# YannDubs/disentangling-vae

Measured on AMD Instinct MI355X. Metric: images/sec (whole node) at 64x64x3, btcvae loss, higher is better.
Workload: dtype f32; 1 GPU; btcvae_celeba (BASELINE.json configs[3]): Burgess VAE 64x64x3, btcvae loss, z=10, tensor handed to _train_iteration B=1024 global (1024 per GPU), Adam lr 0.0005, n_data=202599, fwd+loss+bwd+Adam; batch_per_gpu=1024, global_batch=1024, parallelism=dp1

## Files before the change

disentangling-vae_amd/csrc/conv_up_thin_mm.hip:

```cpp
#include "recon_epilogue.h"

namespace dvae {

#define UTM_ROWS 12
#define UTM_COLS 34
#define UTM_TILE (UTM_ROWS * UTM_COLS * 32)
#define UTM_BR 11
#define UTM_NPOS (UTM_BR * 33)
#define UTM_OR 22
#define UTM_STAGE (3 * UTM_OR * 64)

__device__ __forceinline__ float sigmoid_hw_mm(float v) { return sigmoid_aten(v); }

#ifndef UTM_VARIANT
#define UTM_VARIANT 13
#endif
#ifndef UTM_ABL
#define UTM_ABL 0
#endif
__device__ __forceinline__ void utm_barrier() {
  if (UTM_VARIANT & 4) { wait_lgkmcnt0(); barrier_nofence(); }
  else __syncthreads();
}

template <bool FUSE, int DIST, typename TT>
__global__ __launch_bounds__(512, 4) void k_up_thin_mm(const float* __restrict__ small, const float* __restrict__ wimg,
                                                       const float* __restrict__ bias, float* __restrict__ out, int N,
                                                       int n_units, const TT* __restrict__ target, float* __restrict__ g,
                                                       const float* __restrict__ coef, float* __restrict__ partials) {
  extern __shared__ __attribute__((aligned(16))) float smem[];
  float* tin = smem;
  float* stage = smem + UTM_TILE;
  float* redl = stage + UTM_STAGE;
  float* wl = redl + 8;
  const int tid = threadIdx.x, lane = tid & 63;
  const int wv = __builtin_amdgcn_readfirstlane(tid >> 6);
  const int j = lane & 15, kg = lane >> 4;
  const float gs = FUSE ? coef[DVAE_C_INV_B] : 0.f;
  float lsum = 0.f;

  for (int e = tid; e < UTM_TILE / 4; e += 512) reinterpret_cast<f32x4*>(tin)[e] = f32x4{0.f, 0.f, 0.f, 0.f};

  for (int e = tid; e < 32 * 64 / 4; e += 512) reinterpret_cast<f32x4*>(wl)[e] = reinterpret_cast<const f32x4*>(wimg)[e];
  const float bv = (kg < 3 && bias) ? bias[kg] : 0.f;

  int xb[3], soff[3];
  int key0[3];
  bool x0ok[3], x1ok[3];
#pragma unroll
  for (int s = 0; s < 3; ++s) {
    const int pos0 = 16 * (3 * wv + s) + j;
    const bool pvalid = pos0 < UTM_NPOS;
    const int pos = pvalid ? pos0 : UTM_NPOS - 1;
    const int rq = pos / 33, cq = pos - 33 * rq;
    xb[s] = (rq * UTM_COLS + cq) * 32;
    key0[s] = cq & 7;
    soff[s] = (kg * UTM_OR + 2 * rq) * 64 + 2 * cq - 1;
    x0ok[s] = pvalid && kg < 3 && cq > 0;
    x1ok[s] = pvalid && kg < 3 && cq < 32;
  }
  const bool tile3 = 16 * (3 * wv + 2) < UTM_NPOS;
  const int within = tid & 255, rhalf = tid >> 8;
  const int pgo = rhalf * 1024 + within * 4;
  const int ci_ld = (within >> 3) + 1;
  const int plo = (rhalf * UTM_COLS + ci_ld) * 32 + (((within & 7) ^ (ci_ld & 7)) << 2);
  int bso[3], bgo[3], brow[3];
#pragma unroll
  for (int k = 0; k < 3; ++k) {
    const int e = tid + 512 * k;
    const int c = e / (UTM_OR * 16), rem = e - c * (UTM_OR * 16), r = rem >> 4, x4 = rem & 15;
    brow[k] = e < 3 * UTM_OR * 16 ? r : -1000;
    bso[k] = (c * UTM_OR + r) * 64 + 4 * x4;
    bgo[k] = (c * 64 + r) * 64 + 4 * x4;
  }
  __syncthreads();

  f32x4 pf[6];
  auto load_tile = [&](int unit) {
    const int n = unit / 3, u3 = unit - 3 * n;
    const int sy0 = UTM_BR * u3 - 1;
    const float* base = small + ((long)n * 32 + sy0) * 1024 + pgo;
#pragma unroll
    for (int k = 0; k < 6; ++k) {
      const int sy = sy0 + 2 * k + rhalf;
      pf[k] = f32x4{0.f, 0.f, 0.f, 0.f};
      if (sy >= 0 && sy < 32 && !((UTM_ABL & 16) && N > 0)) pf[k] = *reinterpret_cast<const f32x4*>(base + 2048 * k);
    }
  };
  if ((int)blockIdx.x < n_units) load_tile(blockIdx.x);
  for (int unit = blockIdx.x; unit < n_units; unit += gridDim.x) {
    const int n = unit / 3, u3 = unit - 3 * n;
    const int Y0 = UTM_OR * u3 - 1;
    const long img0 = ((long)n * 3 * 64 + Y0) * 64;
    f32x4 tg[3];
    uchar4 tg8[3];
    auto load_targets_k = [&](int k) {
      const int Y = Y0 + brow[k];
      tg[k] = f32x4{0.f, 0.f, 0.f, 0.f};
      tg8[k] = make_uchar4(0, 0, 0, 0);
      if (Y >= 0 && Y < 64) {
        if constexpr (sizeof(TT) == 4) tg[k] = *reinterpret_cast<const f32x4*>(target + img0 + bgo[k]);
        else tg8[k] = *reinterpret_cast<const uchar4*>(target + img0 + bgo[k]);
      }
    };
    auto load_targets = [&]() {
#pragma unroll
      for (int k = 0; k < 3; ++k) {
        const int Y = Y0 + brow[k];
        tg[k] = f32x4{0.f, 0.f, 0.f, 0.f};
        tg8[k] = make_uchar4(0, 0, 0, 0);
        if (Y >= 0 && Y < 64 && !((UTM_ABL & 4) && N > 0)) {
          if constexpr (sizeof(TT) == 4) tg[k] = *reinterpret_cast<const f32x4*>(target + img0 + bgo[k]);
          else tg8[k] = *reinterpret_cast<const uchar4*>(target + img0 + bgo[k]);
        }
      }
    };
#pragma unroll
    for (int k = 0; k < 6; ++k) *reinterpret_cast<f32x4*>(tin + plo + 2 * UTM_COLS * 32 * k) = pf[k];
    if ((UTM_VARIANT & 1) && unit + (int)gridDim.x < n_units) load_tile(unit + gridDim.x);
    if (FUSE && (UTM_VARIANT & 2)) load_targets();
    if (FUSE && (UTM_VARIANT & 16)) load_targets_k(0);
    utm_barrier();
    f32x4 acc[3];
#pragma unroll
    for (int s = 0; s < 3; ++s) acc[s] = f32x4{0.f, 0.f, 0.f, 0.f};
#pragma unroll
    for (int tap = 0; tap < 4; ++tap) {
      const int a = tap >> 1, b = tap & 1;
      f32x4 x[3][2];
      float wr[8];
#pragma unroll
      for (int i = 0; i < 8; ++i) wr[i] = wl[(tap * 8 + i) * 64 + lane];
#pragma unroll
      for (int s = 0; s < 3; ++s) {
        if (s == 2 && !tile3) continue;
        const int key = (key0[s] + b) & 7;
        const float* px = tin + xb[s] + (a * UTM_COLS + b) * 32;
        x[s][0] = *reinterpret_cast<const f32x4*>(px + (((2 * kg) ^ key) << 2));
        x[s][1] = *reinterpret_cast<const f32x4*>(px + (((2 * kg + 1) ^ key) << 2));
      }
#pragma unroll
      for (int i = 0; i < 8; ++i) {
#pragma unroll
        for (int s = 0; s < 3; ++s) {
          if (s == 2 && !tile3) continue;
          if (!((UTM_ABL & 1) && N > 0)) acc[s] = __builtin_amdgcn_mfma_f32_16x16x4f32(wr[i], x[s][i >> 2][i & 3], acc[s], 0, 0, 0);
        }
      }
    }
    if (FUSE && (UTM_VARIANT & 8)) load_targets();
    if (FUSE && (UTM_VARIANT & 16)) { load_targets_k(1); load_targets_k(2); }
#pragma unroll
    for (int s = 0; s < 3; ++s) {
      if (s == 2 && !tile3) continue;
      float* sp = stage + soff[s];
      if (x0ok[s]) { sp[0] = acc[s][0] + bv; sp[64] = acc[s][2] + bv; }
      if (x1ok[s]) { sp[1] = acc[s][1] + bv; sp[65] = acc[s][3] + bv; }
    }
    utm_barrier();
    if (!(UTM_VARIANT & 1) && unit + (int)gridDim.x < n_units) load_tile(unit + gridDim.x);
    if (FUSE && !(UTM_VARIANT & (2 | 8 | 16))) load_targets();
    if (FUSE && sizeof(TT) != 4) {
#pragma unroll
      for (int k = 0; k < 3; ++k) tg[k] = f32x4{to_unit(tg8[k].x), to_unit(tg8[k].y), to_unit(tg8[k].z), to_unit(tg8[k].w)};
    }
#pragma unroll
    for (int k = 0; k < 3; ++k) {
      const int Y = Y0 + brow[k];
      if (Y < 0 || Y >= 64) continue;
      f32x4 v = *reinterpret_cast<const f32x4*>(stage + bso[k]);
      f32x4 gl = {0.f, 0.f, 0.f, 0.f};
#pragma unroll
      for (int q = 0; q < 4; ++q) {
        if ((UTM_ABL & 2) && N > 0) {
          gl[q] = v[q] + tg[k][q];
        } else if (FUSE && DIST == DVAE_REC_BERNOULLI) {
          float y, glq;
          lsum += sigmoid_bce_logit(v[q], tg[k][q], &y, &glq);
          v[q] = y;
          gl[q] = gs * glq;
        } else {
          const float y = sigmoid_hw_mm(v[q]);
          v[q] = y;
          if (FUSE) {
            float glq, gr;
            lsum += recon_elem(y, tg[k][q], DIST, &glq, &gr);
            gl[q] = gs * glq;
          }
        }
      }
      if ((UTM_ABL & 8) && N > 0) { lsum += v[0] + v[1] + v[2] + v[3] + gl[0] + gl[1] + gl[2] + gl[3]; continue; }
      *reinterpret_cast<f32x4*>(out + img0 + bgo[k]) = v;
      if (FUSE) *reinterpret_cast<f32x4*>(g + img0 + bgo[k]) = gl;
    }
  }
  if (FUSE) {
    const float v = wave_sum(lsum);
    __syncthreads();
    if (lane == 0) redl[wv] = v;
    __syncthreads();
    if (tid == 0) {
      float s = 0.f;
#pragma unroll
      for (int w = 0; w < 8; ++w) s += redl[w];
      partials[blockIdx.x] = s;
    }
    for (int k = gridDim.x + blockIdx.x * 512 + tid; k < DVAE_REC_NPART; k += gridDim.x * 512) partials[k] = 0.f;
  }
}

int launch_up_thin_mm(const float* small, const float* wimg, const float* bias, const void* target, int target_u8, float* out,
                      float* g, int dist, const float* coef, float* partials, int N, int act, hipStream_t s) {
  static const bool off = env_off("DVAE_UP_THIN_MM");
  static const int min_n = env_int("DVAE_UP_THIN_MM_MIN_N", 1);
  if (off || N < min_n || act != DVAE_ACT_SIGMOID) return 1;
  if ((((uintptr_t)small | (uintptr_t)out | (uintptr_t)g) & 15) != 0 || ((uintptr_t)target & (target_u8 ? 3 : 15)) != 0) return 1;
  const int n_units = 3 * N;
  static const int cap = env_int("DVAE_UP_THIN_MM_GRID", 512);
  const int grid = n_units < cap ? n_units : cap;
  constexpr size_t lds = (size_t)(UTM_TILE + UTM_STAGE + 8 + 32 * 64) * sizeof(float);
#define UTM_GO(FUSE_, DIST_, TT_)                                                                                         \
  do {                                                                                                                    \
    static DeviceOnce attr;                                                                                               \
    if (attr.first())                                                                                                     \
      (void)hipFuncSetAttribute((const void*)k_up_thin_mm<FUSE_, DIST_, TT_>, hipFuncAttributeMaxDynamicSharedMemorySize, (int)lds); \
    hipLaunchKernelGGL((k_up_thin_mm<FUSE_, DIST_, TT_>), dim3(grid), dim3(512), lds, s, small, wimg, bias, out, N, n_units,      \
                       (const TT_*)target, g, coef, partials);                                                           \
  } while (0)
  if (!target) UTM_GO(false, 0, float);
  else if (target_u8) {
    if (dist == DVAE_REC_BERNOULLI) UTM_GO(true, DVAE_REC_BERNOULLI, uint8_t);
    else if (dist == DVAE_REC_GAUSSIAN) UTM_GO(true, DVAE_REC_GAUSSIAN, uint8_t);
    else UTM_GO(true, DVAE_REC_LAPLACE, uint8_t);
  } else {
    if (dist == DVAE_REC_BERNOULLI) UTM_GO(true, DVAE_REC_BERNOULLI, float);
    else if (dist == DVAE_REC_GAUSSIAN) UTM_GO(true, DVAE_REC_GAUSSIAN, float);
    else UTM_GO(true, DVAE_REC_LAPLACE, float);
  }
#undef UTM_GO
  DVAE_CHECK_LAUNCH();
  return 0;
}

}
```

Before: 989,600 images/s.

## Stream input tiles into LDS via async DMA and hoist target loads

```diff
diff --git a/disentangling-vae_amd/csrc/conv_up_thin_mm.hip b/disentangling-vae_amd/csrc/conv_up_thin_mm.hip
--- a/disentangling-vae_amd/csrc/conv_up_thin_mm.hip
+++ b/disentangling-vae_amd/csrc/conv_up_thin_mm.hip
@@ -12,16 +12,13 @@
 
 __device__ __forceinline__ float sigmoid_hw_mm(float v) { return sigmoid_aten(v); }
 
-#ifndef UTM_VARIANT
-#define UTM_VARIANT 13
-#endif
+__device__ __attribute__((aligned(16))) float k_utm_zero16[4] = {0.f, 0.f, 0.f, 0.f};
 #ifndef UTM_ABL
 #define UTM_ABL 0
 #endif
-__device__ __forceinline__ void utm_barrier() {
-  if (UTM_VARIANT & 4) { wait_lgkmcnt0(); barrier_nofence(); }
-  else __syncthreads();
-}
+__device__ __forceinline__ void utm_barrier() { wait_lgkmcnt0(); barrier_nofence(); }
+__device__ __forceinline__ void utm_need(f32x4& v) { asm volatile("" : "+v"(v)); }
+__device__ __forceinline__ void utm_need(unsigned& v) { asm volatile("" : "+v"(v)); }
 
 template <bool FUSE, int DIST, typename TT>
 __global__ __launch_bounds__(512, 4) void k_up_thin_mm(const float* __restrict__ small, const float* __restrict__ wimg,
@@ -38,14 +35,11 @@
   const int j = lane & 15, kg = lane >> 4;
   const float gs = FUSE ? coef[DVAE_C_INV_B] : 0.f;
   float lsum = 0.f;
-
   for (int e = tid; e < UTM_TILE / 4; e += 512) reinterpret_cast<f32x4*>(tin)[e] = f32x4{0.f, 0.f, 0.f, 0.f};
-
   for (int e = tid; e < 32 * 64 / 4; e += 512) reinterpret_cast<f32x4*>(wl)[e] = reinterpret_cast<const f32x4*>(wimg)[e];
   const float bv = (kg < 3 && bias) ? bias[kg] : 0.f;
 
-  int xb[3], soff[3];
-  int key0[3];
+  int xb[3], soff[3], key0[3];
   bool x0ok[3], x1ok[3];
 #pragma unroll
   for (int s = 0; s < 3; ++s) {
@@ -60,10 +54,23 @@
     x1ok[s] = pvalid && kg < 3 && cq < 32;
   }
   const bool tile3 = 16 * (3 * wv + 2) < UTM_NPOS;
-  const int within = tid & 255, rhalf = tid >> 8;
-  const int pgo = rhalf * 1024 + within * 4;
-  const int ci_ld = (within >> 3) + 1;
-  const int plo = (rhalf * UTM_COLS + ci_ld) * 32 + (((within & 7) ^ (ci_ld & 7)) << 2);
+  const int dpx = lane >> 3;
+  const int dlo = dpx * 32 + (((lane & 7) ^ ((dpx + 1) & 7)) << 2);
+  const unsigned lds0 = (unsigned)(unsigned long long)(__attribute__((address_space(3))) void*)smem;
+  auto issue_tile = [&](int unit) {
+    if ((UTM_ABL & 16) && N > 0) return;
+    const int n = unit / 3, u3 = unit - 3 * n;
+    const int sy0 = UTM_BR * u3 - 1;
+    const float* base = small + ((long)n * 32 + sy0) * 1024 + dlo;
+#pragma unroll
+    for (int k = 0; k < 6; ++k) {
+      const int d = wv + 8 * k;
+      const int r = d >> 2, c8 = d & 3;
+      const int sy = sy0 + r;
+      const float* src = (sy >= 0 && sy < 32) ? base + r * 1024 + c8 * 256 : k_utm_zero16;
+      lds_dma16(src, __builtin_amdgcn_readfirstlane(lds0 + (unsigned)((r * UTM_COLS + 1 + 8 * c8) * 32) * 4u));
+    }
+  };
   int bso[3], bgo[3], brow[3];
 #pragma unroll
   for (int k = 0; k < 3; ++k) {
@@ -75,52 +82,25 @@
   }
   __syncthreads();
 
-  f32x4 pf[6];
-  auto load_tile = [&](int unit) {
-    const int n = unit / 3, u3 = unit - 3 * n;
-    const int sy0 = UTM_BR * u3 - 1;
-    const float* base = small + ((long)n * 32 + sy0) * 1024 + pgo;
-#pragma unroll
-    for (int k = 0; k < 6; ++k) {
-      const int sy = sy0 + 2 * k + rhalf;
-      pf[k] = f32x4{0.f, 0.f, 0.f, 0.f};
-      if (sy >= 0 && sy < 32 && !((UTM_ABL & 16) && N > 0)) pf[k] = *reinterpret_cast<const f32x4*>(base + 2048 * k);
-    }
-  };
-  if ((int)blockIdx.x < n_units) load_tile(blockIdx.x);
+  if ((int)blockIdx.x < n_units) issue_tile(blockIdx.x);
+  wait_vmcnt<0>();
+  utm_barrier();
   for (int unit = blockIdx.x; unit < n_units; unit += gridDim.x) {
     const int n = unit / 3, u3 = unit - 3 * n;
     const int Y0 = UTM_OR * u3 - 1;
     const long img0 = ((long)n * 3 * 64 + Y0) * 64;
     f32x4 tg[3];
-    uchar4 tg8[3];
-    auto load_targets_k = [&](int k) {
+    unsigned tg8[3];
+#pragma unroll
+    for (int k = 0; k < 3; ++k) {
       const int Y = Y0 + brow[k];
       tg[k] = f32x4{0.f, 0.f, 0.f, 0.f};
-      tg8[k] = make_uchar4(0, 0, 0, 0);
-      if (Y >= 0 && Y < 64) {
+      tg8[k] = 0u;
+      if (FUSE && Y >= 0 && Y < 64 && !((UTM_ABL & 4) && N > 0)) {
         if constexpr (sizeof(TT) == 4) tg[k] = *reinterpret_cast<const f32x4*>(target + img0 + bgo[k]);
-        else tg8[k] = *reinterpret_cast<const uchar4*>(target + img0 + bgo[k]);
-      }
-    };
-    auto load_targets = [&]() {
-#pragma unroll
-      for (int k = 0; k < 3; ++k) {
-        const int Y = Y0 + brow[k];
-        tg[k] = f32x4{0.f, 0.f, 0.f, 0.f};
-        tg8[k] = make_uchar4(0, 0, 0, 0);
-        if (Y >= 0 && Y < 64 && !((UTM_ABL & 4) && N > 0)) {
-          if constexpr (sizeof(TT) == 4) tg[k] = *reinterpret_cast<const f32x4*>(target + img0 + bgo[k]);
-          else tg8[k] = *reinterpret_cast<const uchar4*>(target + img0 + bgo[k]);
-        }
-      }
-    };
-#pragma unroll
-    for (int k = 0; k < 6; ++k) *reinterpret_cast<f32x4*>(tin + plo + 2 * UTM_COLS * 32 * k) = pf[k];
-    if ((UTM_VARIANT & 1) && unit + (int)gridDim.x < n_units) load_tile(unit + gridDim.x);
-    if (FUSE && (UTM_VARIANT & 2)) load_targets();
-    if (FUSE && (UTM_VARIANT & 16)) load_targets_k(0);
-    utm_barrier();
+        else tg8[k] = *reinterpret_cast<const unsigned*>(target + img0 + bgo[k]);
+      }
+    }
     f32x4 acc[3];
 #pragma unroll
     for (int s = 0; s < 3; ++s) acc[s] = f32x4{0.f, 0.f, 0.f, 0.f};
@@ -148,8 +128,6 @@
         }
       }
     }
-    if (FUSE && (UTM_VARIANT & 8)) load_targets();
-    if (FUSE && (UTM_VARIANT & 16)) { load_targets_k(1); load_targets_k(2); }
 #pragma unroll
     for (int s = 0; s < 3; ++s) {
       if (s == 2 && !tile3) continue;
@@ -157,42 +135,59 @@
       if (x0ok[s]) { sp[0] = acc[s][0] + bv; sp[64] = acc[s][2] + bv; }
       if (x1ok[s]) { sp[1] = acc[s][1] + bv; sp[65] = acc[s][3] + bv; }
     }
+    if (FUSE) {
+#pragma unroll
+      for (int k = 0; k < 3; ++k) {
+        if constexpr (sizeof(TT) == 4) utm_need(tg[k]);
+        else utm_need(tg8[k]);
+      }
+    }
     utm_barrier();
-    if (!(UTM_VARIANT & 1) && unit + (int)gridDim.x < n_units) load_tile(unit + gridDim.x);
-    if (FUSE && !(UTM_VARIANT & (2 | 8 | 16))) load_targets();
+    if (unit + (int)gridDim.x < n_units) issue_tile(unit + gridDim.x);
     if (FUSE && sizeof(TT) != 4) {
 #pragma unroll
-      for (int k = 0; k < 3; ++k) tg[k] = f32x4{to_unit(tg8[k].x), to_unit(tg8[k].y), to_unit(tg8[k].z), to_unit(tg8[k].w)};
-    }
+      for (int k = 0; k < 3; ++k)
+        tg[k] = f32x4{to_unit((uint8_t)(tg8[k] & 0xff)), to_unit((uint8_t)((tg8[k] >> 8) & 0xff)), to_unit((uint8_t)((tg8[k] >> 16) & 0xff)),
+                      to_unit((uint8_t)(tg8[k] >> 24))};
+    }
+    f32x4 v[3], gl[3];
+    bool on[3];
 #pragma unroll
     for (int k = 0; k < 3; ++k) {
       const int Y = Y0 + brow[k];
-      if (Y < 0 || Y >= 64) continue;
-      f32x4 v = *reinterpret_cast<const f32x4*>(stage + bso[k]);
-      f32x4 gl = {0.f, 0.f, 0.f, 0.f};
+      on[k] = Y >= 0 && Y < 64;
+      v[k] = gl[k] = f32x4{0.f, 0.f, 0.f, 0.f};
+      if (!on[k]) continue;
+      v[k] = *reinterpret_cast<const f32x4*>(stage + bso[k]);
 #pragma unroll
       for (int q = 0; q < 4; ++q) {
         if ((UTM_ABL & 2) && N > 0) {
-          gl[q] = v[q] + tg[k][q];
+          gl[k][q] = v[k][q] + tg[k][q];
         } else if (FUSE && DIST == DVAE_REC_BERNOULLI) {
           float y, glq;
-          lsum += sigmoid_bce_logit(v[q], tg[k][q], &y, &glq);
-          v[q] = y;
-          gl[q] = gs * glq;
+          lsum += sigmoid_bce_logit(v[k][q], tg[k][q], &y, &glq);
+          v[k][q] = y;
+          gl[k][q] = gs * glq;
         } else {
-          const float y = sigmoid_hw_mm(v[q]);
-          v[q] = y;
+          const float y = sigmoid_hw_mm(v[k][q]);
+          v[k][q] = y;
           if (FUSE) {
             float glq, gr;
             lsum += recon_elem(y, tg[k][q], DIST, &glq, &gr);
-            gl[q] = gs * glq;
+            gl[k][q] = gs * glq;
           }
         }
       }
-      if ((UTM_ABL & 8) && N > 0) { lsum += v[0] + v[1] + v[2] + v[3] + gl[0] + gl[1] + gl[2] + gl[3]; continue; }
-      *reinterpret_cast<f32x4*>(out + img0 + bgo[k]) = v;
-      if (FUSE) *reinterpret_cast<f32x4*>(g + img0 + bgo[k]) = gl;
-    }
+    }
+    wait_vmcnt<0>();
+#pragma unroll
+    for (int k = 0; k < 3; ++k) {
+      if (!on[k]) continue;
+      if ((UTM_ABL & 8) && N > 0) { lsum += v[k][0] + v[k][1] + v[k][2] + v[k][3] + gl[k][0] + gl[k][1] + gl[k][2] + gl[k][3]; continue; }
+      *reinterpret_cast<f32x4*>(out + img0 + bgo[k]) = v[k];
+      if (FUSE) *reinterpret_cast<f32x4*>(g + img0 + bgo[k]) = gl[k];
+    }
+    utm_barrier();
   }
   if (FUSE) {
     const float v = wave_sum(lsum);
```

Result: no change. 996,700 images/s, median of 6 (+0.7%).
